# lmb-freiburg/hand3d

Measured on NVIDIA H100. Metric: images/sec full pipeline 320x320, higher is better.
Workload: dtype bf16 hi/lo split x3 MMA passes, fp32 accumulate (fp32 parity, 1e-3)

## Files before the change

### hand3d_b200/csrc/conv_wgmma.cu

```cuda
#include <cuda.h>

#include <algorithm>
#include <cstdlib>
#include <cstring>
#include <vector>

#include "common.cuh"
#include "split_fmt.cuh"

namespace h3d {

namespace {

constexpr int BM = 128;
constexpr int BK = 64;
constexpr int kThreads = 384;
constexpr int kConsumerThreads = 256;
constexpr int A_TILE_BYTES = BM * BK * 2;
constexpr int STG_COLS = 64;
constexpr int STG_PITCH = STG_COLS + 1;
constexpr int STG_BYTES = BM * STG_PITCH * 4;
constexpr int kSmemBudget = 227 * 1024 - 2048 - STG_BYTES;

__host__ __device__ constexpr int stage_bytes(int BN, int PASSES) { return (PASSES >= 3 ? 2 : 1) * (A_TILE_BYTES + BN * BK * 2); }
__host__ __device__ constexpr int num_stages(int BN, int PASSES) {
    return kSmemBudget / stage_bytes(BN, PASSES) > 8 ? 8 : kSmemBudget / stage_bytes(BN, PASSES);
}
__host__ __device__ constexpr int smem_bytes(int BN, int PASSES) { return num_stages(BN, PASSES) * stage_bytes(BN, PASSES) + STG_BYTES + 2048; }

struct TcParams {
    const float* bias;
    uint16_t* y_hi; uint16_t* y_lo; uint8_t* y_l8; uint8_t* y_h8; int Cy_total, cy_off;
    float corr_scale;
    float* yf; int Cyf_total, cyf_off;
    int B, H, W, k, pad, cin_chunks;
    int TW, TH, TB, tiles_w, tiles_h, n_tiles, num_tiles;
    int n_valid;
    int pool;
    int chunk_kb;
    int leaky;
    int* err_flag;
};

__device__ __forceinline__ uint32_t smem_u32(const void* p) { return (uint32_t)__cvta_generic_to_shared(p); }

__device__ __forceinline__ void mbar_init(uint64_t* bar, uint32_t count) {
    asm volatile("mbarrier.init.shared::cta.b64 [%0], %1;" ::"r"(smem_u32(bar)), "r"(count) : "memory");
}
__device__ __forceinline__ void mbar_expect_tx(uint64_t* bar, uint32_t bytes) {
    asm volatile("mbarrier.arrive.expect_tx.shared::cta.b64 _, [%0], %1;" ::"r"(smem_u32(bar)), "r"(bytes) : "memory");
}
__device__ __forceinline__ void mbar_arrive(uint64_t* bar) {
    asm volatile("mbarrier.arrive.shared::cta.b64 _, [%0];" ::"r"(smem_u32(bar)) : "memory");
}
constexpr uint32_t kTryWaitHintNs = 20000u;
__device__ __forceinline__ bool mbar_try_wait(uint64_t* bar, uint32_t parity) {
    uint32_t ok;
    asm volatile(
        "{\n\t.reg .pred p;\n\t"
        "mbarrier.try_wait.parity.shared::cta.b64 p, [%1], %2, %3;\n\t"
        "selp.u32 %0, 1, 0, p;\n\t}"
        : "=r"(ok) : "r"(smem_u32(bar)), "r"(parity), "r"(kTryWaitHintNs) : "memory");
    return ok != 0;
}
__device__ __forceinline__ void mbar_wait(uint64_t* bar, uint32_t parity, int* err_flag, int code) {
    if (mbar_try_wait(bar, parity)) return;
    const long long t0 = clock64();
    while (!mbar_try_wait(bar, parity)) {
        if (clock64() - t0 > 4000000000ll) {
            if (err_flag) { atomicExch_system(err_flag, code); __threadfence_system(); }
            __trap();
        }
    }
}
__device__ __forceinline__ void tma_load_4d(const CUtensorMap* map, void* dst, uint64_t* bar, int c0, int c1, int c2, int c3) {
    asm volatile(
        "cp.async.bulk.tensor.4d.shared::cluster.global.mbarrier::complete_tx::bytes [%0], [%1, {%3, %4, %5, %6}], [%2];"
        ::"r"(smem_u32(dst)), "l"(reinterpret_cast<uint64_t>(map)), "r"(smem_u32(bar)), "r"(c0), "r"(c1), "r"(c2), "r"(c3)
        : "memory");
}
__device__ __forceinline__ void tma_load_2d(const CUtensorMap* map, void* dst, uint64_t* bar, int c0, int c1) {
    asm volatile(
        "cp.async.bulk.tensor.2d.shared::cluster.global.mbarrier::complete_tx::bytes [%0], [%1, {%3, %4}], [%2];"
        ::"r"(smem_u32(dst)), "l"(reinterpret_cast<uint64_t>(map)), "r"(smem_u32(bar)), "r"(c0), "r"(c1)
        : "memory");
}
template <int N> __device__ __forceinline__ void setmaxnreg_dec() { asm volatile("setmaxnreg.dec.sync.aligned.u32 %0;" ::"n"(N)); }
template <int N> __device__ __forceinline__ void setmaxnreg_inc() { asm volatile("setmaxnreg.inc.sync.aligned.u32 %0;" ::"n"(N)); }
__device__ __forceinline__ void prefetch_tmap(const CUtensorMap* map) {
    asm volatile("prefetch.tensormap [%0];" ::"l"(reinterpret_cast<uint64_t>(map)) : "memory");
}

__device__ __forceinline__ void pdl_launch_dependents() { asm volatile("griddepcontrol.launch_dependents;" ::: "memory"); }
__device__ __forceinline__ void pdl_wait() { asm volatile("griddepcontrol.wait;" ::: "memory"); }

__device__ __forceinline__ bool elect_one() {
    uint32_t pred;
    asm volatile("{\n\t.reg .pred p;\n\telect.sync _|p, 0xffffffff;\n\tselp.u32 %0, 1, 0, p;\n\t}" : "=r"(pred));
    return pred != 0;
}
__device__ __forceinline__ void cluster_sync_all() {
    asm volatile("barrier.cluster.arrive.release.aligned;" ::: "memory");
    asm volatile("barrier.cluster.wait.acquire.aligned;" ::: "memory");
}
__device__ __forceinline__ uint32_t cluster_ctarank() { uint32_t r; asm volatile("mov.u32 %0, %%cluster_ctarank;" : "=r"(r)); return r; }
__device__ __forceinline__ void fence_proxy_async_smem() { asm volatile("fence.proxy.async.shared::cta;" ::: "memory"); }
__device__ __forceinline__ void named_bar_sync(int id, int threads) { asm volatile("bar.sync %0, %1;" ::"r"(id), "r"(threads) : "memory"); }
__device__ __forceinline__ uint32_t sw128_chunk(int r, int c) { return (uint32_t)(r * 128 + ((c ^ (r & 7)) << 4)); }

__device__ __forceinline__ uint64_t desc_sw128(uint32_t saddr) {
    return (uint64_t)((saddr & 0x3FFFFu) >> 4) | (1ull << 16) | (64ull << 32) | (1ull << 62);
}
__device__ __forceinline__ uint64_t desc_sw64(uint32_t saddr) {
    return (uint64_t)((saddr & 0x3FFFFu) >> 4) | (1ull << 16) | (32ull << 32) | (2ull << 62);
}
__device__ __forceinline__ void wgmma_fence() { asm volatile("wgmma.fence.sync.aligned;" ::: "memory"); }
__device__ __forceinline__ void wgmma_commit() { asm volatile("wgmma.commit_group.sync.aligned;" ::: "memory"); }
template <int N> __device__ __forceinline__ void wgmma_wait() { asm volatile("wgmma.wait_group.sync.aligned %0;" ::"n"(N) : "memory"); }
template <int NR> __device__ __forceinline__ void fence_regs(float* d) {
#pragma unroll
    for (int i = 0; i < NR; ++i) asm volatile("" : "+f"(d[i])::"memory");
}

// ... 193 lines not shown
        if (PASSES == 4) {
            tma_load_4d(x_lo, st + A_TILE_BYTES, fb, a0, a1, a2, a3);
            tma_load_4d(x_h8, st + A_TILE_BYTES + C::A8_TILE_BYTES, fb, a0, a1, a2, a3);
            tma_load_2d(w_lo, st + 2 * A_TILE_BYTES + C::B_TILE_BYTES, fb, kcol, n0);
            tma_load_2d(w_l8, st + 2 * A_TILE_BYTES + C::B_TILE_BYTES + C::B8_TILE_BYTES, fb, kcol, n0);
        }
    }
    __syncwarp();
    if (++r.stage == C::STAGES) { r.stage = 0; r.phase ^= 1; }
}

template <int BN, int PASSES, bool FP16>
__device__ __forceinline__ void mma_tile(Ring& r, int kblocks, int chunk_kb, float* racc, int wg, int lane, int* err_flag) {
    using C = RingCfg<BN, PASSES>;
    constexpr int NR = BN / 2;
    constexpr int NR8 = PASSES == 4 ? NR : 1;
    float acc[NR], acc8[NR8];
#pragma unroll
    for (int i = 0; i < NR; ++i) acc[i] = 0.f;
#pragma unroll
    for (int i = 0; i < NR8; ++i) acc8[i] = 0.f;
    for (int kb0 = 0; kb0 < kblocks; kb0 += chunk_kb) {
        const int kb1 = min(kblocks, kb0 + chunk_kb);
        int pend = -1;
        for (int kb = kb0; kb < kb1; ++kb) {
            mbar_wait(&r.full[r.stage], r.phase, err_flag, 3);
            const uint32_t sa = smem_u32(r.base + r.stage * C::STAGE_BYTES);
            const uint32_t a_rows = (uint32_t)wg * 64 * 128;
            const uint64_t a_hi = desc_sw128(sa + a_rows);
            const uint64_t a_lo = desc_sw128(sa + A_TILE_BYTES + a_rows);
            const uint64_t b_hi = desc_sw128(sa + (PASSES >= 3 ? 2 : 1) * A_TILE_BYTES);
            const uint64_t b_lo = desc_sw128(sa + 2 * A_TILE_BYTES + C::B_TILE_BYTES);
            fence_regs<NR>(acc);
            fence_regs<NR8>(acc8);
            wgmma_fence();
#pragma unroll
            for (int j = 0; j < BK / 16; ++j) {
                const uint64_t koff = (uint64_t)j * 2;
                mma16<BN, FP16>(acc, a_hi + koff, b_hi + koff, (uint32_t)((kb > kb0) | (j != 0)));
                if (PASSES == 3) {
                    mma16<BN, FP16>(acc, a_hi + koff, b_lo + koff, 1u);
                    mma16<BN, FP16>(acc, a_lo + koff, b_hi + koff, 1u);
                }
            }
            if (PASSES == 4) {
                const uint32_t a8_rows = (uint32_t)wg * 64 * 64;
                const uint64_t a_l8 = desc_sw64(sa + A_TILE_BYTES + a8_rows);
                const uint64_t a_h8 = desc_sw64(sa + A_TILE_BYTES + C::A8_TILE_BYTES + a8_rows);
                const uint64_t b_h8 = desc_sw64(sa + 2 * A_TILE_BYTES + C::B_TILE_BYTES);
                const uint64_t b_l8 = desc_sw64(sa + 2 * A_TILE_BYTES + C::B_TILE_BYTES + C::B8_TILE_BYTES);
#pragma unroll
                for (int j = 0; j < 2; ++j) {
                    const uint64_t koff = (uint64_t)j * 2;
                    mma8<BN>(acc8, a_l8 + koff, b_h8 + koff, (uint32_t)((kb > kb0) | (j != 0)));
                    mma8<BN>(acc8, a_h8 + koff, b_l8 + koff, 1u);
                }
            }
            wgmma_commit();
            fence_regs<NR>(acc);
            fence_regs<NR8>(acc8);
            wgmma_wait<1>();
            if (pend >= 0 && lane == 0) mbar_arrive(&r.empty[pend]);
            pend = r.stage;
            if (++r.stage == C::STAGES) { r.stage = 0; r.phase ^= 1; }
        }
        wgmma_wait<0>();
        if (lane == 0) mbar_arrive(&r.empty[pend]);
        fence_regs<NR>(acc);
        fence_regs<NR8>(acc8);
        if constexpr (PASSES == 4) {
#pragma unroll
            for (int i = 0; i < NR; ++i) acc[i] += acc8[i];
        }
        if (kb0 == 0) {
#pragma unroll
            for (int i = 0; i < NR; ++i) racc[i] = acc[i];
        } else {
#pragma unroll
            for (int i = 0; i < NR; ++i) racc[i] += acc[i];
        }
    }
}

template <int BN, int PASSES, bool FP16, class PixOf>
__device__ __forceinline__ void store_tile(const TcParams& p, const float* racc, float* stg, int ct, int n0, PixOf pix_of) {
    const int wg = ct >> 7, tt = ct & 127;
    const int r0 = wg * 64 + (tt >> 5) * 16 + ((tt & 31) >> 2);
    const int cq = 2 * (tt & 3);
    const int row = ct & 127, half = ct >> 7;
    int64_t pix; bool valid;
    pix_of(row, pix, valid);
#pragma unroll
    for (int rnd = 0; rnd < BN / STG_COLS; ++rnd) {
        named_bar_sync(1, kConsumerThreads);
#pragma unroll
        for (int j = 0; j < STG_COLS / 8; ++j) {
            const int jj = rnd * (STG_COLS / 8) + j, c = 8 * j + cq;
            stg[r0 * STG_PITCH + c] = racc[4 * jj];
            stg[r0 * STG_PITCH + c + 1] = racc[4 * jj + 1];
            stg[(r0 + 8) * STG_PITCH + c] = racc[4 * jj + 2];
            stg[(r0 + 8) * STG_PITCH + c + 1] = racc[4 * jj + 3];
        }
        named_bar_sync(1, kConsumerThreads);
        float f[32];
#pragma unroll
        for (int q = 0; q < 32; ++q) f[q] = stg[row * STG_PITCH + half * 32 + q];
        epilogue_store32<PASSES, FP16>(p, f, pix, n0 + rnd * STG_COLS + half * 32, valid);
    }
}

constexpr int kProducerRegs = 40, kConsumerRegs = 232;

template <int BN, int PASSES, bool FP16>
__global__ void __launch_bounds__(kThreads, 1)
conv_tc_kernel(const __grid_constant__ CUtensorMap map_x_hi, const __grid_constant__ CUtensorMap map_x_lo,
               const __grid_constant__ CUtensorMap map_w_hi, const __grid_constant__ CUtensorMap map_w_lo,
               const __grid_constant__ CUtensorMap map_x_h8, const __grid_constant__ CUtensorMap map_w_l8, const TcParams p) {
    using C = RingCfg<BN, PASSES>;
    static_assert(PASSES != 4 || FP16, "fp8-correction mode uses an fp16 main plane");
    static_assert(smem_bytes(BN, PASSES) <= 227 * 1024, "conv_tc_kernel: shared memory budget");

    extern __shared__ __align__(1024) uint8_t smem_raw[];
    uint8_t* smem = reinterpret_cast<uint8_t*>((reinterpret_cast<uintptr_t>(smem_raw) + 1023) & ~(uintptr_t)1023);
    float* stg = reinterpret_cast<float*>(smem + C::STAGES * C::STAGE_BYTES);
    uint64_t* bars = reinterpret_cast<uint64_t*>(smem + C::STAGES * C::STAGE_BYTES + STG_BYTES);
    Ring ring{smem, bars, bars + C::STAGES, 0, 0};

    const int warp = threadIdx.x >> 5, lane = threadIdx.x & 31;
    const int wg = __shfl_sync(0xFFFFFFFFu, (int)threadIdx.x / 128, 0);
    const int kblocks = p.k * p.k * p.cin_chunks;

    if (threadIdx.x == 0) {
        prefetch_tmap(&map_x_hi); prefetch_tmap(&map_w_hi);
        if (PASSES >= 3) { prefetch_tmap(&map_x_lo); prefetch_tmap(&map_w_lo); }
        if (PASSES == 4) { prefetch_tmap(&map_x_h8); prefetch_tmap(&map_w_l8); }
        for (int s = 0; s < C::STAGES; ++s) { mbar_init(&ring.full[s], 1); mbar_init(&ring.empty[s], kConsumerThreads / 32); }
        asm volatile("fence.mbarrier_init.release.cluster;" ::: "memory");
    }
    __syncthreads();
    pdl_launch_dependents();
    pdl_wait();

    if (wg == 0) {
        setmaxnreg_dec<kProducerRegs>();
        if (warp == 0) {
            for (int tile = blockIdx.x; tile < p.num_tiles; tile += gridDim.x) {
                const int nt = tile % p.n_tiles, mt = tile / p.n_tiles;
                const int tw = mt % p.tiles_w, th = (mt / p.tiles_w) % p.tiles_h, tb = mt / (p.tiles_w * p.tiles_h);
                const int w0 = tw * p.TW - p.pad, h0 = th * p.TH - p.pad, b0 = tb * p.TB, n0 = nt * BN;
                int kcol = 0;
                for (int kh = 0; kh < p.k; ++kh)
                    for (int kw = 0; kw < p.k; ++kw)
                        for (int cc = 0; cc < p.cin_chunks; ++cc, kcol += BK)
                            produce_kblock<BN, PASSES>(ring, &map_x_hi, &map_x_lo, &map_x_h8, &map_w_hi, &map_w_lo, &map_w_l8, cc * BK,
                                                       w0 + kw, h0 + kh, b0, kcol, n0, p.err_flag);
            }
        }
    } else {
        setmaxnreg_inc<kConsumerRegs>();
        const int ct = threadIdx.x - 128;
        float racc[BN / 2];
        for (int tile = blockIdx.x; tile < p.num_tiles; tile += gridDim.x) {
            const int nt = tile % p.n_tiles, mt = tile / p.n_tiles;
            const int tw = mt % p.tiles_w, th = (mt / p.tiles_w) % p.tiles_h, tb = mt / (p.tiles_w * p.tiles_h);
            mma_tile<BN, PASSES, FP16>(ring, kblocks, p.chunk_kb, racc, ct >> 7, lane, p.err_flag);
            store_tile<BN, PASSES, FP16>(p, racc, stg, ct, nt * BN, [&](int row, int64_t& pix, bool& valid) {
                const int w_l = row % p.TW, h_l = (row / p.TW) % p.TH, b_l = row / (p.TW * p.TH);
                const int w = tw * p.TW + w_l, h = th * p.TH + h_l, b = tb * p.TB + b_l;
                valid = (w < p.W) && (h < p.H) && (b < p.B);
                pix = ((int64_t)b * p.H + h) * p.W + w;
                if (p.pool) {
                    const int par = p.pool == 2 ? 1 : 0;
                    valid = valid && ((w & 1) == par) && ((h & 1) == par);
                    pix = ((int64_t)b * (p.H >> 1) + (h >> 1)) * (p.W >> 1) + (w >> 1);
                }
            });
        }
    }
}

constexpr int C3_TW = 16, C3_TH = 8;
constexpr int C3T_THREADS = 256;
constexpr int C3T_B_BYTES = 128 * BK * 2;
constexpr int C3T_PW = C3_TW + 2, C3T_PH = C3_TH + 2;
constexpr int C3T_PATCH_FLOATS = C3T_PH * C3T_PW * 3;
constexpr int C3T_SMEM = C3T_B_BYTES + 2 * A_TILE_BYTES + STG_BYTES + C3T_PATCH_FLOATS * 4 + 1024 ;

template <bool FP16>
__global__ void __launch_bounds__(C3T_THREADS, 2)
conv_c3_tc_kernel(const float* __restrict__ x, const float* __restrict__ w, const TcParams p) {
    extern __shared__ __align__(1024) uint8_t smem_raw[];
    uint8_t* smem = reinterpret_cast<uint8_t*>((reinterpret_cast<uintptr_t>(smem_raw) + 1023) & ~(uintptr_t)1023);
    uint8_t* bsm = smem;
    uint8_t* asm_ = smem + C3T_B_BYTES;
    float* stg = reinterpret_cast<float*>(asm_ + 2 * A_TILE_BYTES);
    float* patch = stg + BM * STG_PITCH;

    const int t = threadIdx.x, wg = t >> 7;
    if (t < 128) {
        const int co = t & 63;
        uint32_t pk[16];
#pragma unroll
        for (int k2 = 0; k2 < 16; ++k2) {
            float v0 = 0.f, v1 = 0.f;
            if (2 * k2 < 27) v0 = __ldg(w + (2 * k2) * 64 + co);
            if (2 * k2 + 1 < 27) v1 = __ldg(w + (2 * k2 + 1) * 64 + co);
            const uint32_t h = pack_hi2<FP16>(v0, v1);
            if (t < 64) pk[k2] = h;
            else { const float2 r = unpack2<FP16>(h); pk[k2] = pack_hi2<FP16>(v0 - r.x, v1 - r.y); }
        }
#pragma unroll
        for (int c = 0; c < 4; ++c)
            *reinterpret_cast<uint4*>(bsm + sw128_chunk(t, c)) = make_uint4(pk[4 * c], pk[4 * c + 1], pk[4 * c + 2], pk[4 * c + 3]);
    }
    pdl_launch_dependents();
    pdl_wait();

    const uint32_t sb = smem_u32(bsm), sa = smem_u32(asm_);
    const uint64_t b_hi = desc_sw128(sb), b_lo = desc_sw128(sb + 64 * 128);
    const uint64_t a_hi = desc_sw128(sa + wg * 64 * 128), a_lo = desc_sw128(sa + A_TILE_BYTES + wg * 64 * 128);
    for (int tile = blockIdx.x; tile < p.num_tiles; tile += gridDim.x) {
        const int tw = tile % p.tiles_w, th = (tile / p.tiles_w) % p.tiles_h, b = tile / (p.tiles_w * p.tiles_h);
        {
            const int x0 = tw * C3_TW - 1, y0 = th * C3_TH - 1;
            const float* xb = x + (int64_t)b * p.H * p.W * 3;
            for (int i = t; i < C3T_PATCH_FLOATS; i += C3T_THREADS) {
                const int r = i / (C3T_PW * 3), rem = i - r * (C3T_PW * 3);
                const int gy = y0 + r, gx = x0 + rem / 3;
                float v = 0.f;
                if (gy >= 0 && gy < p.H && gx >= 0 && gx < p.W) v = __ldg(xb + ((int64_t)gy * p.W + x0) * 3 + rem);
                patch[i] = v;
            }
        }
        __syncthreads();
        if (t < 128) {
            const int w_l = t % C3_TW, h_l = t / C3_TW;
            uint32_t hi[16], lo[16];
#pragma unroll
            for (int k2 = 0; k2 < 16; ++k2) {
                float v0 = 0.f, v1 = 0.f;
                if (2 * k2 < 27) { const int k = 2 * k2; v0 = patch[(h_l + k / 9) * (C3T_PW * 3) + w_l * 3 + (k % 9)]; }
                if (2 * k2 + 1 < 27) { const int k = 2 * k2 + 1; v1 = patch[(h_l + k / 9) * (C3T_PW * 3) + w_l * 3 + (k % 9)]; }
                hi[k2] = pack_hi2<FP16>(v0, v1);
                const float2 r = unpack2<FP16>(hi[k2]);
                lo[k2] = pack_hi2<FP16>(v0 - r.x, v1 - r.y);
            }
#pragma unroll
            for (int c = 0; c < 4; ++c) {
// ... 124 lines not shown
                if (P.rot && lane < 9) P.rot[9 * b + lane] = R[lane];
                const bool right = P.hand_side[2 * b + 1] > P.hand_side[2 * b];
                for (int i = lane; i < 63; i += 32) {
                    float c3[3];
                    const int kp = i / 3;
                    c3[0] = __ldcg(P.can + 63 * b + 3 * kp); c3[1] = __ldcg(P.can + 63 * b + 3 * kp + 1); c3[2] = __ldcg(P.can + 63 * b + 3 * kp + 2);
                    const int j = i - kp * 3;
                    const float cz = right ? -c3[2] : c3[2];
                    P.out[63 * b + i] = c3[0] * R[j] + c3[1] * R[3 + j] + cz * R[6 + j];
                }
            }
        }
    }
    cluster_sync_all();
}

typedef CUresult (*EncodeTiledFn)(CUtensorMap*, CUtensorMapDataType, cuuint32_t, void*, const cuuint64_t*, const cuuint64_t*,
                                  const cuuint32_t*, const cuuint32_t*, CUtensorMapInterleave, CUtensorMapSwizzle,
                                  CUtensorMapL2promotion, CUtensorMapFloatOOBfill);

EncodeTiledFn get_encode_fn() {
    static EncodeTiledFn fn = nullptr;
    if (fn) return fn;
    void* ptr = nullptr;
    cudaDriverEntryPointQueryResult qres;
    cudaError_t e = cudaGetDriverEntryPoint("cuTensorMapEncodeTiled", &ptr, cudaEnableDefault, &qres);
    if (e != cudaSuccess || qres != cudaDriverEntryPointSuccess || !ptr) {
        set_error("cuTensorMapEncodeTiled not available (%s)", cudaGetErrorString(e));
        return nullptr;
    }
    fn = reinterpret_cast<EncodeTiledFn>(ptr);
    return fn;
}

bool encode_act_map(CUtensorMap* m, const void* base, int C_total, int C_used, int W, int H, int B, int TW, int TH, int TB, int es = 2) {
    EncodeTiledFn fn = get_encode_fn();
    if (!fn) return false;
    cuuint64_t dims[4] = {(cuuint64_t)C_used, (cuuint64_t)W, (cuuint64_t)H, (cuuint64_t)B};
    cuuint64_t strides[3] = {(cuuint64_t)C_total * es, (cuuint64_t)W * C_total * es, (cuuint64_t)H * W * C_total * es};
    cuuint32_t box[4] = {(cuuint32_t)BK, (cuuint32_t)TW, (cuuint32_t)TH, (cuuint32_t)TB};
    cuuint32_t estr[4] = {1, 1, 1, 1};
    CUresult r = fn(m, es == 2 ? CU_TENSOR_MAP_DATA_TYPE_UINT16 : CU_TENSOR_MAP_DATA_TYPE_UINT8, 4, const_cast<void*>(base), dims, strides,
                    box, estr, CU_TENSOR_MAP_INTERLEAVE_NONE, es == 2 ? CU_TENSOR_MAP_SWIZZLE_128B : CU_TENSOR_MAP_SWIZZLE_64B,
                    CU_TENSOR_MAP_L2_PROMOTION_L2_256B, CU_TENSOR_MAP_FLOAT_OOB_FILL_NONE);
    if (r != CUDA_SUCCESS) { set_error("cuTensorMapEncodeTiled(activations) failed: %d", (int)r); return false; }
    return true;
}

bool encode_w_map(CUtensorMap* m, const void* base, int Ktot, int Cout_pad, int BN, int es = 2) {
    EncodeTiledFn fn = get_encode_fn();
    if (!fn) return false;
    cuuint64_t dims[2] = {(cuuint64_t)Ktot, (cuuint64_t)Cout_pad};
    cuuint64_t strides[1] = {(cuuint64_t)Ktot * es};
    cuuint32_t box[2] = {(cuuint32_t)BK, (cuuint32_t)BN};
    cuuint32_t estr[2] = {1, 1};
    CUresult r = fn(m, es == 2 ? CU_TENSOR_MAP_DATA_TYPE_UINT16 : CU_TENSOR_MAP_DATA_TYPE_UINT8, 2, const_cast<void*>(base), dims, strides,
                    box, estr, CU_TENSOR_MAP_INTERLEAVE_NONE, es == 2 ? CU_TENSOR_MAP_SWIZZLE_128B : CU_TENSOR_MAP_SWIZZLE_64B,
                    CU_TENSOR_MAP_L2_PROMOTION_L2_256B, CU_TENSOR_MAP_FLOAT_OOB_FILL_NONE);
    if (r != CUDA_SUCCESS) { set_error("cuTensorMapEncodeTiled(weights) failed: %d", (int)r); return false; }
    return true;
}

void choose_tile(int B, int H, int W, int* TW, int* TH, int* TB, bool pool = false) {
    static const int cand[][3] = {{16, 8, 1}, {8, 16, 1}, {32, 4, 1}, {4, 32, 1}, {64, 2, 1}, {128, 1, 1}, {8, 8, 2},
                                  {16, 4, 2}, {4, 16, 2}, {8, 4, 4}, {4, 8, 4}, {4, 4, 8}, {8, 2, 8}, {2, 2, 32}, {1, 1, 128}};
    int64_t best = -1;
    for (auto& c : cand) {
        if (pool && !((c[0] % 2) == 0 && c[0] <= 16 && (c[1] % 2) == 0)) continue;
        const int64_t tiles = (int64_t)ceil_div(W, c[0]) * ceil_div(H, c[1]) * ceil_div(B, c[2]);
        if (best < 0 || tiles < best) { best = tiles; *TW = c[0]; *TH = c[1]; *TB = c[2]; }
    }
}

template <int BN, int PASSES, bool FP16>
int launch_inst(const TcConvPlan* pl, cudaStream_t s);

}

struct TcConvPlan {
    int device = 0;
    TcConvDesc d;
    CUtensorMap map_x_hi, map_x_lo, map_w_hi, map_w_lo, map_x_h8, map_w_l8;
    TcParams p;
    int BN, grid;
};

constexpr int kMaxDevices = 64;
static int current_device() { int dev = 0; if (cudaGetDevice(&dev) != cudaSuccess) { cudaGetLastError(); dev = 0; } return dev; }
int tc_num_sms() {
    static int n[kMaxDevices] = {};
    const int dev = current_device() % kMaxDevices;
    if (!n[dev]) {
        int v = 0;
        if (cudaDeviceGetAttribute(&v, cudaDevAttrMultiProcessorCount, dev) != cudaSuccess || v <= 0) { cudaGetLastError(); v = 132; }
        n[dev] = v;
    }
    return n[dev];
}
template <typename K>
static int smem_opt_in(K kernel, int bytes, bool* done ) {
    const int dev = current_device() % kMaxDevices;
    if (!done[dev]) {
        H3D_CUDA(cudaFuncSetAttribute(kernel, cudaFuncAttributeMaxDynamicSharedMemorySize, bytes));
        done[dev] = true;
    }
    return H3D_OK;
}

template <typename... KArgs, typename... Args>
static cudaError_t launch_pdl(void (*kernel)(KArgs...), dim3 grid, dim3 block, size_t smem, cudaStream_t s, Args&&... args) {
    cudaLaunchConfig_t cfg = {};
    cfg.gridDim = grid; cfg.blockDim = block; cfg.dynamicSmemBytes = smem; cfg.stream = s;
    cudaLaunchAttribute attr[1];
    attr[0].id = cudaLaunchAttributeProgrammaticStreamSerialization;
    attr[0].val.programmaticStreamSerializationAllowed = tc_tuning().pdl ? 1 : 0;
    cfg.attrs = attr; cfg.numAttrs = 1;
    return cudaLaunchKernelEx(&cfg, kernel, static_cast<KArgs>(args)...);
}

TcTuning& tc_tuning() {
    static TcTuning t = [] {
        TcTuning v;
        auto geti = [](const char* n, int d) { const char* e = getenv(n); return e ? atoi(e) : d; };
        v.two_cta = geti("H3D_TC_2CTA", -1);
        v.bn = geti("H3D_TC_BN", 0);
        v.c64 = geti("H3D_TC_C64", 1);
        v.c64x2 = geti("H3D_TC_C64X2", 1);
        v.pair128 = geti("H3D_TC_PAIR128", 1);
        v.stack = geti("H3D_TC_STACK", 1);
        v.chunk_kb = geti("H3D_TC_CHUNK_KB", 0);
        v.exp = geti("H3D_TC_EXP", 0);
        v.no_side_stream = geti("H3D_NO_SIDE_STREAM", 0);
        v.no_pool_fusion = geti("H3D_NO_POOL_FUSION", 0);
        v.lift_direct = geti("H3D_LIFT_DIRECT", 0);
        v.c3_ffma = geti("H3D_C3_FFMA", 0);
        v.c3_tma = geti("H3D_C3_TMA", 1);
        v.pdl = geti("H3D_PDL", 1);
        v.fc_chain = geti("H3D_FC_CHAIN", 1);
        v.c64_tma_out = geti("H3D_C64_TMA_OUT", 1);
        v.chain = geti("H3D_TC_CHAIN", 1);
        v.small_batch_split = geti("H3D_TC_SMALL_SPLIT", 1);
        v.fuse_c1 = geti("H3D_FUSE_C1", 1);
        v.no_seg_fusion = geti("H3D_NO_SEG_FUSION", 0);
        return v;
    }();
    return t;
}
int tc_set_tuning(const char* key, int value) {
    TcTuning& t = tc_tuning();
    const std::string k(key ? key : "");
    if (k == "tc_2cta") t.two_cta = value;
    else if (k == "tc_bn") t.bn = value;
    else if (k == "tc_c64") t.c64 = value;
    else if (k == "tc_c64x2") t.c64x2 = value;
    else if (k == "tc_pair128") t.pair128 = value;
    else if (k == "tc_stack") t.stack = value;
    else if (k == "tc_chunk_kb") t.chunk_kb = value;
    else if (k == "tc_exp") t.exp = value;
    else if (k == "no_side_stream") t.no_side_stream = value;
    else if (k == "no_pool_fusion") t.no_pool_fusion = value;
    else if (k == "lift_direct") t.lift_direct = value;
    else if (k == "c3_ffma") t.c3_ffma = value;
    else if (k == "c3_tma") t.c3_tma = value;
    else if (k == "pdl") t.pdl = value;
    else if (k == "fc_chain") t.fc_chain = value;
    else if (k == "c64_tma_out") t.c64_tma_out = value;
    else if (k == "tc_chain") t.chain = value;
    else if (k == "tc_small_split") t.small_batch_split = value;
    else if (k == "fuse_c1") t.fuse_c1 = value;
    else if (k == "no_seg_fusion") t.no_seg_fusion = value;
    else { set_error("h3d_set_tuning: unknown key '%s'", k.c_str()); return H3D_EINVAL; }
    return H3D_OK;
}

namespace {
template <int BN, int PASSES, bool FP16>
int launch_inst(const TcConvPlan* pl, cudaStream_t s) {
    constexpr int smem = smem_bytes(BN, PASSES);
    static bool attr[kMaxDevices] = {};
    if (int rc = smem_opt_in(conv_tc_kernel<BN, PASSES, FP16>, smem, attr)) return rc;
    H3D_CUDA(launch_pdl(conv_tc_kernel<BN, PASSES, FP16>, dim3(pl->grid), dim3(kThreads), smem, s, pl->map_x_hi, pl->map_x_lo, pl->map_w_hi,
                        pl->map_w_lo, pl->map_x_h8, pl->map_w_l8, pl->p));
    return H3D_OK;
}
}

TcConvPlan* tc_conv_plan_create(const TcConvDesc& d) {
    if (d.Cin_pad % BK != 0 || d.Cout_pad % 64 != 0 || (d.k != 1 && d.k != 3 && d.k != 5 && d.k != 7) || (d.passes != 1 && d.passes != 3 && d.passes != 4)) {
        set_error("tc_conv: unsupported geometry (Cin_pad=%d Cout_pad=%d k=%d passes=%d)", d.Cin_pad, d.Cout_pad, d.k, d.passes);
        return nullptr;
    }
    const bool padded_out = d.Cout % 32 != 0;
    if (d.y.hi && ((d.Cy_total % 8) || (d.cy_off % 8))) { set_error("tc_conv: split output channel offset/stride must be multiples of 8"); return nullptr; }
    if (d.yf && !padded_out && ((d.Cyf_total % 4) || (d.cyf_off % 4))) { set_error("tc_conv: fp32 output channel offset/stride must be multiples of 4"); return nullptr; }
    if (padded_out && d.pool == 1) { set_error("tc_conv: fused pooling needs Cout %% 32 == 0"); return nullptr; }
    if (d.pool < 0 || d.pool > 2) { set_error("tc_conv: pool mode must be 0 (none), 1 (max-pool) or 2 (stride 2)"); return nullptr; }
    if (d.pool == 2 && d.k < 3) { set_error("tc_conv: stride 2 needs k >= 3 (for k = 1 TF's 'SAME' samples the even pixels, not the odd ones)"); return nullptr; }
    if (d.c1_w) { set_error("tc_conv: conv1_1 is not fused into conv1_2 on sm_90a (tc_conv_can_fuse_first is false)"); return nullptr; }
    if (d.passes == 3 && (!d.x.lo || !d.w.lo)) { set_error("tc_conv: 3-pass mode needs lo planes"); return nullptr; }
    if (d.passes == 4 && (!d.x.l8 || !d.x.h8 || !d.w.l8 || !d.w.h8 || d.half != Half16::FP16 || d.corr_scale <= 0.f)) {
        set_error("tc_conv: fp8-correction mode needs fp16 + e4m3 l8/h8 planes for activations and weights and a correction scale");
        return nullptr;
    }
    if (d.passes == 4 && d.y.hi && (!d.y.l8 || !d.y.h8)) { set_error("tc_conv: fp8-correction mode needs l8/h8 output planes"); return nullptr; }
    if (d.passes == 4 && d.y.hi && ((d.Cy_total % 16) || (d.cy_off % 16))) { set_error("tc_conv: fp8 planes need 16-channel aligned offsets"); return nullptr; }
    if (d.pool && ((d.H | d.W) & 1)) { set_error("tc_conv: fused max-pool / stride 2 needs even H and W"); return nullptr; }
    TcConvPlan* pl = new TcConvPlan();
    pl->d = d;
    const TcTuning& tune = tc_tuning();
    int BN = d.Cout_pad % 128 == 0 ? 128 : 64;
    if ((int64_t)d.H * d.W <= 256) BN = 64;
    if ((tune.bn == 64 || tune.bn == 128) && d.Cout_pad % tune.bn == 0) BN = tune.bn;
    if (d.passes == 4) BN = 64;
    int TW, TH, TB;
    choose_tile(d.B, d.H, d.W, &TW, &TH, &TB, d.pool == 1);
    pl->BN = BN;
    pl->device = current_device();
    TcParams& p = pl->p;
    p.bias = d.bias;
    p.y_hi = d.y.hi; p.y_lo = d.y.lo; p.y_l8 = d.y.l8; p.y_h8 = d.y.h8; p.Cy_total = d.Cy_total; p.cy_off = d.cy_off;
    p.corr_scale = d.corr_scale;
    p.yf = d.yf; p.Cyf_total = d.Cyf_total; p.cyf_off = d.cyf_off;
    p.B = d.B; p.H = d.H; p.W = d.W; p.k = d.k; p.pad = d.k / 2; p.cin_chunks = d.Cin_pad / BK;
    p.TW = TW; p.TH = TH; p.TB = TB;
    p.tiles_w = ceil_div(d.W, TW); p.tiles_h = ceil_div(d.H, TH);
    p.n_tiles = d.Cout_pad / BN;
    p.num_tiles = p.tiles_w * p.tiles_h * ceil_div(d.B, TB) * p.n_tiles;
    p.leaky = d.leaky;
    p.n_valid = d.Cout;
    p.pool = d.pool;
    p.err_flag = d.err_flag;
    p.chunk_kb = d.passes >= 3 ? 9 : 27;
    if (tune.chunk_kb > 0) p.chunk_kb = tune.chunk_kb;
    pl->grid = std::min(p.num_tiles, tc_num_sms());
    const int Ktot = d.k * d.k * d.Cin_pad;
    bool ok = encode_act_map(&pl->map_x_hi, d.x.hi, d.Cin_total, d.Cin_pad, d.W, d.H, d.B, TW, TH, TB) &&
              encode_w_map(&pl->map_w_hi, d.w.hi, Ktot, d.Cout_pad, BN);
    if (ok && d.passes == 3)
        ok = encode_act_map(&pl->map_x_lo, d.x.lo, d.Cin_total, d.Cin_pad, d.W, d.H, d.B, TW, TH, TB) &&
             encode_w_map(&pl->map_w_lo, d.w.lo, Ktot, d.Cout_pad, BN);
    if (ok && d.passes == 4)
        ok = encode_act_map(&pl->map_x_lo, d.x.l8, d.Cin_total, d.Cin_pad, d.W, d.H, d.B, TW, TH, TB, 1) &&
             encode_act_map(&pl->map_x_h8, d.x.h8, d.Cin_total, d.Cin_pad, d.W, d.H, d.B, TW, TH, TB, 1) &&
             encode_w_map(&pl->map_w_lo, d.w.h8, Ktot, d.Cout_pad, BN, 1) &&
             encode_w_map(&pl->map_w_l8, d.w.l8, Ktot, d.Cout_pad, BN, 1);
    if (ok && d.passes == 1) { pl->map_x_lo = pl->map_x_hi; pl->map_w_lo = pl->map_w_hi; }
    if (ok && d.passes != 4) { pl->map_x_h8 = pl->map_x_hi; pl->map_w_l8 = pl->map_w_hi; }
    if (!ok) { delete pl; return nullptr; }
    return pl;
}

void tc_conv_plan_destroy(TcConvPlan* p) { delete p; }

bool tc_conv_plan_chainable(const TcConvPlan*) { return false; }
int tc_conv_plan_signal_target(const TcConvPlan* p) { return p->p.tiles_w * p->p.tiles_h * p->p.n_tiles; }
const TcConvDesc& tc_conv_plan_desc(const TcConvPlan* p) { return p->d; }
void tc_conv_plan_set_chain(TcConvPlan*, int*, const int*, int, int*) {}

int64_t tc_conv_flops(const TcConvPlan* p) {
    return 2ll * p->d.B * p->d.H * p->d.W * p->d.k * p->d.k * (int64_t)p->d.Cin_pad * p->d.Cout_pad;
}

bool tc_conv_can_fuse_first(int, int, int, int, int, int, int) { return false; }

int tc_conv_launch_image(const TcConvPlan*, const float*, cudaStream_t) {
    set_error("tc_conv_launch_image: conv1_1 is not fused into conv1_2 on sm_90a");
    return H3D_EINVAL;
}

int tc_conv_launch(const TcConvPlan* pl, cudaStream_t s) {
    const bool fp16 = pl->d.half == Half16::FP16;
    const int key = pl->BN * 10 + pl->d.passes;
#define CASE(BN_, P_)                                                                  \
    case BN_ * 10 + P_:                                                                \
        return fp16 ? launch_inst<BN_, P_, true>(pl, s) : launch_inst<BN_, P_, false>(pl, s);
    switch (key) {
        CASE(64, 1) CASE(64, 3) CASE(128, 1) CASE(128, 3)
        case 64 * 10 + 4: return launch_inst<64, 4, true>(pl, s);
    }
#undef CASE
    set_error("tc_conv: no kernel instance for BN=%d passes=%d", pl->BN, pl->d.passes);
    return H3D_EINVAL;
}

int launch_conv_c3_tc(const float* x, const float* w, const float* bias, Split y, int Cs_total, int cs_off, int B, int H, int W, int leaky,
                      Half16 half, cudaStream_t s, int* err_flag) {
    H3D_REQUIRE(x && w && bias && y.hi && !y.l8 && (Cs_total % 8) == 0 && (cs_off % 8) == 0, "conv_c3_tc: bad argument");
    TcParams p{};
    p.bias = bias;
    p.y_hi = y.hi; p.y_lo = y.lo; p.Cy_total = Cs_total; p.cy_off = cs_off;
    p.corr_scale = 1.f;
    p.B = B; p.H = H; p.W = W; p.k = 3; p.pad = 1; p.cin_chunks = 1;
    p.TW = C3_TW; p.TH = C3_TH; p.TB = 1;
    p.tiles_w = ceil_div(W, C3_TW); p.tiles_h = ceil_div(H, C3_TH); p.n_tiles = 1;
    p.num_tiles = p.tiles_w * p.tiles_h * B;
    p.n_valid = 64; p.pool = 0; p.chunk_kb = 1; p.leaky = leaky; p.err_flag = err_flag;
    const int grid = std::min(p.num_tiles, 2 * tc_num_sms());
    static bool attr_h[kMaxDevices] = {}, attr_b[kMaxDevices] = {};
    if (int rc = smem_opt_in(conv_c3_tc_kernel<true>, C3T_SMEM, attr_h)) return rc;
    if (int rc = smem_opt_in(conv_c3_tc_kernel<false>, C3T_SMEM, attr_b)) return rc;
    if (half == Half16::FP16) H3D_CUDA(launch_pdl(conv_c3_tc_kernel<true>, dim3(grid), dim3(C3T_THREADS), (size_t)C3T_SMEM, s, x, w, p));
    else H3D_CUDA(launch_pdl(conv_c3_tc_kernel<false>, dim3(grid), dim3(C3T_THREADS), (size_t)C3T_SMEM, s, x, w, p));
    return H3D_OK;
}

struct FcChainPlan { FcChainParams P; Half16 half; int grid; };

FcChainPlan* fc_chain_plan_create(const FcChainDesc* chains, int num_chains, int B, Half16 half, const float* can, const float* uxyz,
                                  unsigned int* counter, int* err_flag) {
    if (num_chains < 1 || num_chains > 2 || B < 1) { set_error("fc_chain: bad geometry"); return nullptr; }
    FcChainPlan* pl = new FcChainPlan();
    memset(&pl->P, 0, sizeof(pl->P));
    pl->half = half; pl->grid = num_chains * kFcCluster;
    FcChainParams& P = pl->P;
    P.num_chains = num_chains; P.B = B; P.can = can; P.uxyz = uxyz; P.counter = counter; P.err_flag = err_flag;
    for (int c = 0; c < num_chains; ++c) {
        const FcChainDesc& cd = chains[c];
        if (cd.num_layers < 1 || cd.num_layers > kFcMaxLayers) { set_error("fc_chain: 1..4 layers per chain"); delete pl; return nullptr; }
        P.chain[c].num_layers = cd.num_layers;
        for (int l = 0; l < cd.num_layers; ++l) {
            const FcLayerDesc& d = cd.layer[l];
            FcLayer& L = P.chain[c].layer[l];
            const int Kpad = (int)align_up(d.in_features, BK);
            if (!d.x.hi || !d.x.lo || !d.w.hi || !d.w.lo || d.out_pad % 64 || d.x_stride < Kpad || (d.y.hi && (d.y_stride % 8))) {
                set_error("fc_chain: bad layer %d of chain %d", l, c); delete pl; return nullptr;
            }
// ... 35 lines not shown
```

Before: 991.6.

## Load tall activation halo once per kw/cin chunk and reuse across kh taps

For 3-pass convs, activations and weights now use separate smem rings. A single TMA box of TH+k-1 rows is loaded per (kw, cin chunk) and reused for all kh taps by shifting the wgmma descriptor row offset, with the loop order changed to kw, cc, kh. This cuts activation TMA traffic by about a factor of k and frees smem for more weight stages. In exchange, descriptor addressing becomes more complex, smem size is computed at runtime, and weights-only stages can become the bottleneck.

```diff
diff --git a/hand3d_b200/csrc/conv_wgmma.cu b/hand3d_b200/csrc/conv_wgmma.cu
--- a/hand3d_b200/csrc/conv_wgmma.cu
+++ b/hand3d_b200/csrc/conv_wgmma.cu
@@ -20,7 +20,8 @@
 constexpr int STG_COLS = 64;
 constexpr int STG_PITCH = STG_COLS + 1;
 constexpr int STG_BYTES = BM * STG_PITCH * 4;
-constexpr int kSmemBudget = 227 * 1024 - 2048 - STG_BYTES;
+constexpr int kMaxSmem = 227 * 1024;
+constexpr int kSmemBudget = kMaxSmem - 2048 - STG_BYTES;
 
 __host__ __device__ constexpr int stage_bytes(int BN, int PASSES) { return (PASSES >= 3 ? 2 : 1) * (A_TILE_BYTES + BN * BK * 2); }
 __host__ __device__ constexpr int num_stages(int BN, int PASSES) {
@@ -39,6 +40,9 @@
     int pool;
     int chunk_kb;
     int leaky;
+    int a_tall;
+    int a_rows;
+    int a_slots, b_slots;
     int* err_flag;
 };
 
@@ -398,6 +402,143 @@
     }
 }
 
+struct Slots {
+    uint8_t* base;
+    uint64_t* full;
+    uint64_t* empty;
+    int n, bytes;
+    int stage;
+    uint32_t phase;
+    __device__ __forceinline__ uint8_t* slot() const { return base + stage * bytes; }
+    __device__ __forceinline__ void advance() { if (++stage == n) { stage = 0; phase ^= 1; } }
+};
+__host__ __device__ constexpr int a_row_bytes(int PASSES) { return PASSES == 1 ? 128 : 256; }
+__host__ __device__ constexpr int b_slot_bytes(int BN, int PASSES) { return (PASSES >= 3 ? 2 : 1) * BN * BK * 2; }
+
+
+template <int BN, int PASSES>
+__device__ __forceinline__ void produce_conv_tile(const TcParams& p, Slots& ra, Slots& rb, const CUtensorMap* x_hi, const CUtensorMap* x_lo,
+                                                  const CUtensorMap* x_h8, const CUtensorMap* w_hi, const CUtensorMap* w_lo,
+                                                  const CUtensorMap* w_l8, int w0, int h0, int b0, int n0) {
+    using C = RingCfg<BN, PASSES>;
+    const int a_plane = p.a_rows * 128;
+    auto kblock = [&](int kh, int kw, int cc) {
+        if (kh == 0 || !p.a_tall) {
+            mbar_wait(&ra.empty[ra.stage], ra.phase ^ 1, p.err_flag, 1);
+            if (elect_one()) {
+                uint8_t* st = ra.slot();
+                uint64_t* fb = &ra.full[ra.stage];
+                const int h = p.a_tall ? h0 : h0 + kh;
+                mbar_expect_tx(fb, ra.bytes);
+                tma_load_4d(x_hi, st, fb, cc * BK, w0 + kw, h, b0);
+                if (PASSES >= 3) tma_load_4d(x_lo, st + a_plane, fb, cc * BK, w0 + kw, h, b0);
+                if (PASSES == 4) tma_load_4d(x_h8, st + a_plane + a_plane / 2, fb, cc * BK, w0 + kw, h, b0);
+            }
+            __syncwarp();
+            ra.advance();
+        }
+        mbar_wait(&rb.empty[rb.stage], rb.phase ^ 1, p.err_flag, 1);
+        if (elect_one()) {
+            uint8_t* st = rb.slot();
+            uint64_t* fb = &rb.full[rb.stage];
+            const int kcol = ((kh * p.k + kw) * p.cin_chunks + cc) * BK;
+            mbar_expect_tx(fb, rb.bytes);
+            tma_load_2d(w_hi, st, fb, kcol, n0);
+            if (PASSES >= 3) tma_load_2d(w_lo, st + C::B_TILE_BYTES, fb, kcol, n0);
+            if (PASSES == 4) tma_load_2d(w_l8, st + C::B_TILE_BYTES + C::B8_TILE_BYTES, fb, kcol, n0);
+        }
+        __syncwarp();
+        rb.advance();
+    };
+    for (int kw = 0; kw < p.k; ++kw)
+        for (int cc = 0; cc < p.cin_chunks; ++cc)
+            for (int kh = 0; kh < p.k; ++kh) kblock(kh, kw, cc);
+}
+
+template <int BN, int PASSES, bool FP16>
+__device__ __forceinline__ void mma_conv_tile(const TcParams& p, Slots& ra, Slots& rb, float* racc, int wg, int a_row0, int lane) {
+    using C = RingCfg<BN, PASSES>;
+    constexpr int NR = BN / 2;
+    constexpr int NR8 = PASSES == 4 ? NR : 1;
+    const int kblocks = p.k * p.k * p.cin_chunks;
+    const uint32_t a_plane = (uint32_t)p.a_rows * 128;
+    float acc[NR], acc8[NR8];
+#pragma unroll
+    for (int i = 0; i < NR; ++i) acc[i] = 0.f;
+#pragma unroll
+    for (int i = 0; i < NR8; ++i) acc8[i] = 0.f;
+    int kh = 0;
+    for (int kb0 = 0; kb0 < kblocks; kb0 += p.chunk_kb) {
+        const int kb1 = min(kblocks, kb0 + p.chunk_kb);
+        int pend_a = -1, pend_b = -1;
+        for (int kb = kb0; kb < kb1; ++kb) {
+            if (kh == 0 || !p.a_tall) mbar_wait(&ra.full[ra.stage], ra.phase, p.err_flag, 3);
+            mbar_wait(&rb.full[rb.stage], rb.phase, p.err_flag, 3);
+            const uint32_t row = p.a_tall ? (uint32_t)(a_row0 + kh * p.TW) : (uint32_t)wg * 64;
+            const uint32_t sa = smem_u32(ra.slot()), sb = smem_u32(rb.slot());
+            const uint64_t a_hi = desc_sw128(sa + row * 128);
+            const uint64_t a_lo = desc_sw128(sa + a_plane + row * 128);
+            const uint64_t b_hi = desc_sw128(sb);
+            const uint64_t b_lo = desc_sw128(sb + C::B_TILE_BYTES);
+            fence_regs<NR>(acc);
+            fence_regs<NR8>(acc8);
+            wgmma_fence();
+#pragma unroll
+            for (int j = 0; j < BK / 16; ++j) {
+                const uint64_t koff = (uint64_t)j * 2;
+                mma16<BN, FP16>(acc, a_hi + koff, b_hi + koff, (uint32_t)((kb > kb0) | (j != 0)));
+                if (PASSES == 3) {
+                    mma16<BN, FP16>(acc, a_hi + koff, b_lo + koff, 1u);
+                    mma16<BN, FP16>(acc, a_lo + koff, b_hi + koff, 1u);
+                }
+            }
+            if (PASSES == 4) {
+                const uint64_t a_l8 = desc_sw64(sa + a_plane + row * 64);
+                const uint64_t a_h8 = desc_sw64(sa + a_plane + a_plane / 2 + row * 64);
+                const uint64_t b_h8 = desc_sw64(sb + C::B_TILE_BYTES);
+                const uint64_t b_l8 = desc_sw64(sb + C::B_TILE_BYTES + C::B8_TILE_BYTES);
+#pragma unroll
+                for (int j = 0; j < 2; ++j) {
+                    const uint64_t koff = (uint64_t)j * 2;
+                    mma8<BN>(acc8, a_l8 + koff, b_h8 + koff, (uint32_t)((kb > kb0) | (j != 0)));
+                    mma8<BN>(acc8, a_h8 + koff, b_l8 + koff, 1u);
+                }
+            }
+            wgmma_commit();
+            fence_regs<NR>(acc);
+            fence_regs<NR8>(acc8);
+            wgmma_wait<1>();
+            if (lane == 0) {
+                if (pend_b >= 0) mbar_arrive(&rb.empty[pend_b]);
+                if (pend_a >= 0) mbar_arrive(&ra.empty[pend_a]);
+            }
+            pend_b = rb.stage;
+            rb.advance();
+            pend_a = -1;
+            if (kh == p.k - 1 || !p.a_tall) { pend_a = ra.stage; ra.advance(); }
+            if (++kh == p.k) kh = 0;
+        }
+        wgmma_wait<0>();
+        if (lane == 0) {
+            mbar_arrive(&rb.empty[pend_b]);
+            if (pend_a >= 0) mbar_arrive(&ra.empty[pend_a]);
+        }
+        fence_regs<NR>(acc);
+        fence_regs<NR8>(acc8);
+        if constexpr (PASSES == 4) {
+#pragma unroll
+            for (int i = 0; i < NR; ++i) acc[i] += acc8[i];
+        }
+        if (kb0 == 0) {
+#pragma unroll
+            for (int i = 0; i < NR; ++i) racc[i] = acc[i];
+        } else {
+#pragma unroll
+            for (int i = 0; i < NR; ++i) racc[i] += acc[i];
+        }
+    }
+}
+
 template <int BN, int PASSES, bool FP16, class PixOf>
 __device__ __forceinline__ void store_tile(const TcParams& p, const float* racc, float* stg, int ct, int n0, PixOf pix_of) {
     const int wg = ct >> 7, tt = ct & 127;
@@ -432,25 +573,35 @@
 conv_tc_kernel(const __grid_constant__ CUtensorMap map_x_hi, const __grid_constant__ CUtensorMap map_x_lo,
                const __grid_constant__ CUtensorMap map_w_hi, const __grid_constant__ CUtensorMap map_w_lo,
                const __grid_constant__ CUtensorMap map_x_h8, const __grid_constant__ CUtensorMap map_w_l8, const TcParams p) {
+    static_assert(PASSES != 4 || FP16, "fp8-correction mode uses an fp16 main plane");
+
+    constexpr bool kTwoRings = PASSES == 3;
     using C = RingCfg<BN, PASSES>;
-    static_assert(PASSES != 4 || FP16, "fp8-correction mode uses an fp16 main plane");
-    static_assert(smem_bytes(BN, PASSES) <= 227 * 1024, "conv_tc_kernel: shared memory budget");
-
     extern __shared__ __align__(1024) uint8_t smem_raw[];
     uint8_t* smem = reinterpret_cast<uint8_t*>((reinterpret_cast<uintptr_t>(smem_raw) + 1023) & ~(uintptr_t)1023);
-    float* stg = reinterpret_cast<float*>(smem + C::STAGES * C::STAGE_BYTES);
-    uint64_t* bars = reinterpret_cast<uint64_t*>(smem + C::STAGES * C::STAGE_BYTES + STG_BYTES);
+    const int a_bytes = p.a_rows * a_row_bytes(PASSES);
+    constexpr int b_bytes = b_slot_bytes(BN, PASSES);
+    uint8_t* b_base = smem + p.a_slots * a_bytes;
+    const int ring_bytes = kTwoRings ? p.a_slots * a_bytes + p.b_slots * b_bytes : C::STAGES * C::STAGE_BYTES;
+    float* stg = reinterpret_cast<float*>(smem + ring_bytes);
+    uint64_t* bars = reinterpret_cast<uint64_t*>(smem + ring_bytes + STG_BYTES);
+    Slots ra{smem, bars, bars + p.a_slots, p.a_slots, a_bytes, 0, 0};
+    Slots rb{b_base, bars + 2 * p.a_slots, bars + 2 * p.a_slots + p.b_slots, p.b_slots, b_bytes, 0, 0};
     Ring ring{smem, bars, bars + C::STAGES, 0, 0};
 
     const int warp = threadIdx.x >> 5, lane = threadIdx.x & 31;
     const int wg = __shfl_sync(0xFFFFFFFFu, (int)threadIdx.x / 128, 0);
-    const int kblocks = p.k * p.k * p.cin_chunks;
 
     if (threadIdx.x == 0) {
         prefetch_tmap(&map_x_hi); prefetch_tmap(&map_w_hi);
         if (PASSES >= 3) { prefetch_tmap(&map_x_lo); prefetch_tmap(&map_w_lo); }
         if (PASSES == 4) { prefetch_tmap(&map_x_h8); prefetch_tmap(&map_w_l8); }
-        for (int s = 0; s < C::STAGES; ++s) { mbar_init(&ring.full[s], 1); mbar_init(&ring.empty[s], kConsumerThreads / 32); }
+        if (kTwoRings) {
+            for (int s = 0; s < p.a_slots; ++s) { mbar_init(&ra.full[s], 1); mbar_init(&ra.empty[s], kConsumerThreads / 32); }
+            for (int s = 0; s < p.b_slots; ++s) { mbar_init(&rb.full[s], 1); mbar_init(&rb.empty[s], kConsumerThreads / 32); }
+        } else {
+            for (int s = 0; s < C::STAGES; ++s) { mbar_init(&ring.full[s], 1); mbar_init(&ring.empty[s], kConsumerThreads / 32); }
+        }
         asm volatile("fence.mbarrier_init.release.cluster;" ::: "memory");
     }
     __syncthreads();
@@ -464,22 +615,29 @@
                 const int nt = tile % p.n_tiles, mt = tile / p.n_tiles;
                 const int tw = mt % p.tiles_w, th = (mt / p.tiles_w) % p.tiles_h, tb = mt / (p.tiles_w * p.tiles_h);
                 const int w0 = tw * p.TW - p.pad, h0 = th * p.TH - p.pad, b0 = tb * p.TB, n0 = nt * BN;
-                int kcol = 0;
-                for (int kh = 0; kh < p.k; ++kh)
-                    for (int kw = 0; kw < p.k; ++kw)
-                        for (int cc = 0; cc < p.cin_chunks; ++cc, kcol += BK)
-                            produce_kblock<BN, PASSES>(ring, &map_x_hi, &map_x_lo, &map_x_h8, &map_w_hi, &map_w_lo, &map_w_l8, cc * BK,
-                                                       w0 + kw, h0 + kh, b0, kcol, n0, p.err_flag);
+                if constexpr (kTwoRings) {
+                    produce_conv_tile<BN, PASSES>(p, ra, rb, &map_x_hi, &map_x_lo, &map_x_h8, &map_w_hi, &map_w_lo, &map_w_l8, w0, h0, b0, n0);
+                } else {
+                    int kcol = 0;
+                    for (int kh = 0; kh < p.k; ++kh)
+                        for (int kw = 0; kw < p.k; ++kw)
+                            for (int cc = 0; cc < p.cin_chunks; ++cc, kcol += BK)
+                                produce_kblock<BN, PASSES>(ring, &map_x_hi, &map_x_lo, &map_x_h8, &map_w_hi, &map_w_lo, &map_w_l8, cc * BK,
+                                                           w0 + kw, h0 + kh, b0, kcol, n0, p.err_flag);
+                }
             }
         }
     } else {
         setmaxnreg_inc<kConsumerRegs>();
         const int ct = threadIdx.x - 128;
+        const int m0 = (ct >> 7) * 64, img = p.TW * p.TH;
+        const int a_row0 = m0 / img * p.TW * (p.TH + p.k - 1) + m0 % img;
         float racc[BN / 2];
         for (int tile = blockIdx.x; tile < p.num_tiles; tile += gridDim.x) {
             const int nt = tile % p.n_tiles, mt = tile / p.n_tiles;
             const int tw = mt % p.tiles_w, th = (mt / p.tiles_w) % p.tiles_h, tb = mt / (p.tiles_w * p.tiles_h);
-            mma_tile<BN, PASSES, FP16>(ring, kblocks, p.chunk_kb, racc, ct >> 7, lane, p.err_flag);
+            if constexpr (kTwoRings) mma_conv_tile<BN, PASSES, FP16>(p, ra, rb, racc, ct >> 7, a_row0, lane);
+            else mma_tile<BN, PASSES, FP16>(ring, p.k * p.k * p.cin_chunks, p.chunk_kb, racc, ct >> 7, lane, p.err_flag);
             store_tile<BN, PASSES, FP16>(p, racc, stg, ct, nt * BN, [&](int row, int64_t& pix, bool& valid) {
                 const int w_l = row % p.TW, h_l = (row / p.TW) % p.TH, b_l = row / (p.TW * p.TH);
                 const int w = tw * p.TW + w_l, h = th * p.TH + h_l, b = tb * p.TB + b_l;
@@ -770,7 +928,7 @@
     TcConvDesc d;
     CUtensorMap map_x_hi, map_x_lo, map_w_hi, map_w_lo, map_x_h8, map_w_l8;
     TcParams p;
-    int BN, grid;
+    int BN, grid, smem;
 };
 
 constexpr int kMaxDevices = 64;
@@ -864,10 +1022,9 @@
 namespace {
 template <int BN, int PASSES, bool FP16>
 int launch_inst(const TcConvPlan* pl, cudaStream_t s) {
-    constexpr int smem = smem_bytes(BN, PASSES);
     static bool attr[kMaxDevices] = {};
-    if (int rc = smem_opt_in(conv_tc_kernel<BN, PASSES, FP16>, smem, attr)) return rc;
-    H3D_CUDA(launch_pdl(conv_tc_kernel<BN, PASSES, FP16>, dim3(pl->grid), dim3(kThreads), smem, s, pl->map_x_hi, pl->map_x_lo, pl->map_w_hi,
+    if (int rc = smem_opt_in(conv_tc_kernel<BN, PASSES, FP16>, kMaxSmem, attr)) return rc;
+    H3D_CUDA(launch_pdl(conv_tc_kernel<BN, PASSES, FP16>, dim3(pl->grid), dim3(kThreads), pl->smem, s, pl->map_x_hi, pl->map_x_lo, pl->map_w_hi,
                         pl->map_w_lo, pl->map_x_h8, pl->map_w_l8, pl->p));
     return H3D_OK;
 }
@@ -921,15 +1078,27 @@
     p.chunk_kb = d.passes >= 3 ? 9 : 27;
     if (tune.chunk_kb > 0) p.chunk_kb = tune.chunk_kb;
     pl->grid = std::min(p.num_tiles, tc_num_sms());
+    const int row_bytes = a_row_bytes(d.passes), b_bytes = b_slot_bytes(BN, d.passes);
+    p.a_tall = d.passes == 3 && TW % 8 == 0 && TW * TH >= 64 && 2 * TW * (TH + d.k - 1) * TB * row_bytes + 3 * b_bytes <= kSmemBudget;
+    const int box_h = p.a_tall ? TH + d.k - 1 : TH;
+    p.a_rows = TW * box_h * TB;
+    const int a_bytes = p.a_rows * row_bytes;
+    if (p.a_tall && d.k > 1) {
+        p.a_slots = 2;
+        p.b_slots = std::min(8, (kSmemBudget - 2 * a_bytes) / b_bytes);
+    } else {
+        p.a_slots = p.b_slots = std::min(8, kSmemBudget / (a_bytes + b_bytes));
+    }
+    pl->smem = d.passes == 3 ? p.a_slots * a_bytes + p.b_slots * b_bytes + STG_BYTES + 2048 : smem_bytes(BN, d.passes);
     const int Ktot = d.k * d.k * d.Cin_pad;
-    bool ok = encode_act_map(&pl->map_x_hi, d.x.hi, d.Cin_total, d.Cin_pad, d.W, d.H, d.B, TW, TH, TB) &&
+    bool ok = encode_act_map(&pl->map_x_hi, d.x.hi, d.Cin_total, d.Cin_pad, d.W, d.H, d.B, TW, box_h, TB) &&
               encode_w_map(&pl->map_w_hi, d.w.hi, Ktot, d.Cout_pad, BN);
     if (ok && d.passes == 3)
-        ok = encode_act_map(&pl->map_x_lo, d.x.lo, d.Cin_total, d.Cin_pad, d.W, d.H, d.B, TW, TH, TB) &&
+        ok = encode_act_map(&pl->map_x_lo, d.x.lo, d.Cin_total, d.Cin_pad, d.W, d.H, d.B, TW, box_h, TB) &&
              encode_w_map(&pl->map_w_lo, d.w.lo, Ktot, d.Cout_pad, BN);
     if (ok && d.passes == 4)
-        ok = encode_act_map(&pl->map_x_lo, d.x.l8, d.Cin_total, d.Cin_pad, d.W, d.H, d.B, TW, TH, TB, 1) &&
-             encode_act_map(&pl->map_x_h8, d.x.h8, d.Cin_total, d.Cin_pad, d.W, d.H, d.B, TW, TH, TB, 1) &&
+        ok = encode_act_map(&pl->map_x_lo, d.x.l8, d.Cin_total, d.Cin_pad, d.W, d.H, d.B, TW, box_h, TB, 1) &&
+             encode_act_map(&pl->map_x_h8, d.x.h8, d.Cin_total, d.Cin_pad, d.W, d.H, d.B, TW, box_h, TB, 1) &&
              encode_w_map(&pl->map_w_lo, d.w.h8, Ktot, d.Cout_pad, BN, 1) &&
              encode_w_map(&pl->map_w_l8, d.w.l8, Ktot, d.Cout_pad, BN, 1);
     if (ok && d.passes == 1) { pl->map_x_lo = pl->map_x_hi; pl->map_w_lo = pl->map_w_hi; }
```

Measured after the change: 1015, median of 6. 1.02x the previous value.
